# oppo-us-research/PoP-Net

Measured on AMD Instinct MI355X. Metric: depth-frames/sec end-to-end (480x640), higher is better.
Workload: dtype bf16

## Files before the change

popnet_amd/csrc/bb64_kernel.h:

```cpp
#pragma once
#include "conv3_kernel.h"


#define BB_INQ (12 * 32 * 32)
#define BB_IN (4 * BB_INQ)
#define BB_MIDQ (10 * 32 * 32)
#define BB_MID (4 * BB_MIDQ)
#define BB_ASLOT 4096
#define BB_OFF_MID (2 * BB_IN)
#define BB_OFF_A (BB_OFF_MID + BB_MID)
#define BB_NSLOT 6
#define BB_LDS (BB_OFF_A + BB_NSLOT * BB_ASLOT)

typedef __attribute__((ext_vector_type(2))) float f32x2;
typedef __attribute__((ext_vector_type(2))) __bf16 bf16x2;
typedef __attribute__((ext_vector_type(2))) short i16x2;
__device__ __forceinline__ unsigned bb_relu_pk(unsigned w) {
    return __builtin_bit_cast(unsigned, __builtin_elementwise_max(__builtin_bit_cast(i16x2, w), i16x2{0, 0}));
}

template <int HV>
__global__ __launch_bounds__((4 * HV + 4) * 64, 1) void bb64_kernel(const BBProblem P) {
    typedef __bf16 T;
    constexpr int CT = 4 / HV, NCW = 4 * HV, NP = CT / 2, PT1 = 5, PT2 = 4, KK = 9, BQ = 6;
    extern __shared__ __attribute__((aligned(16))) char smem[];
    const int tid = threadIdx.x;
    const int lane = tid & 63;
    const int wave = __builtin_amdgcn_readfirstlane(tid >> 6);
    const int c = lane & 15, q = lane >> 4;
    const int W = P.W, H = P.H;

    volatile int *s_tile = reinterpret_cast<volatile int *>(smem + BB_OFF_MID + 31 * 32);
    const bool dyn = P.tickets != nullptr;
    auto next_tile = [&](int t, int k) -> int { return dyn ? __builtin_amdgcn_readfirstlane(s_tile[(k + 1) & 3]) : t + (int)gridDim.x; };
    auto next_tile_raw = [&](int t, int k) -> int { return dyn ? s_tile[(k + 1) & 3] : t + (int)gridDim.x; };
    auto tile_geom = [&](int t, int &b, int &oy0, int &ox0, int &R, int &Wc) {
        b = t / P.tiles_per_img;
        const int rem = t - b * P.tiles_per_img;
        const int ty = rem / P.tiles_x, tx = rem - ty * P.tiles_x;
        oy0 = ty * 8; ox0 = tx * P.Wt;
        R = min(8, H - oy0); Wc = min(P.Wt, W - ox0);
    };

    if (wave >= NCW) {
        const int lw = wave - NCW;
        const unsigned lane16 = (unsigned)lane * 16u;
        int t = blockIdx.x;
        if (t >= P.ntiles) return;
        if (lw < 2) {
            const char *wsrc = (const char *)P.wpack + lw * 2048;
            auto dma_a = [&](int kstep) {
                pn_glds16_s<0>(wsrc + (size_t)kstep * BB_ASLOT, lane16, (unsigned)(BB_OFF_A + (kstep % BB_NSLOT) * BB_ASLOT) + (unsigned)__builtin_amdgcn_readfirstlane(lw * 2048));
                pn_glds16_s<0>(wsrc + (size_t)kstep * BB_ASLOT + 1024, lane16, (unsigned)(BB_OFF_A + (kstep % BB_NSLOT) * BB_ASLOT + 1024) + (unsigned)__builtin_amdgcn_readfirstlane(lw * 2048));
            };
            dma_a(0); dma_a(1); dma_a(2); dma_a(3);
            asm volatile("s_waitcnt vmcnt(0)\n\ts_barrier" ::: "memory");
            asm volatile("s_barrier" ::: "memory");
            for (int k = 0; t < P.ntiles; ++k) {
                const int tnx = next_tile_raw(t, k);
#pragma clang loop unroll(full)
                for (int p = 0; p < 18; ++p) {
                    dma_a((2 * p + 4) % 36);
                    dma_a((2 * p + 5) % 36);
                    asm volatile("s_waitcnt vmcnt(2)\n\ts_barrier" ::: "memory");
                    if (p == 8) asm volatile("s_barrier" ::: "memory");
                }
                asm volatile("s_barrier" ::: "memory");
                t = __builtin_amdgcn_readfirstlane(tnx);
            }
            asm volatile("s_waitcnt vmcnt(0)" ::: "memory");
            return;
        }
        auto dma_in = [&](int tt, int buf, int n) {
            int b, oy0, ox0, R, Wc;
            tile_geom(tt, b, oy0, ox0, R, Wc);
            const int qu = n / 12, row = n % 12;
            const int px = lane >> 1;
            const int iy = oy0 - 2 + row, ix = ox0 - 2 + px;
            const size_t frame_b = ((size_t)b * H * W * P.in_cs + P.in_coff) * 2;
            const bool inb = px < Wc + 4 && (unsigned)ix < (unsigned)W && (unsigned)iy < (unsigned)H;
            const unsigned off = inb ? (unsigned)((iy * W + ix) * P.in_cs * 2 + qu * 32 + (lane & 1) * 16) : P.in_zero_off - (unsigned)frame_b;
            pn_glds16_s<0>((const char *)P.in + frame_b, off, (unsigned)__builtin_amdgcn_readfirstlane(buf * BB_IN + qu * BB_INQ + row * 1024));
        };
        const int n0 = (lw - 2) * 24;
        const bool ticketer = dyn && lw == 2 && lane == 0;
        int ticket = 0;
        auto claim = [&]() -> int { return 2 * (int)gridDim.x + atomicAdd(P.tickets, 1); };
        if (ticketer) ticket = t + (int)gridDim.x;
#pragma unroll
        for (int j = 0; j < 24; ++j) dma_in(t, 0, n0 + j);
        asm volatile("s_waitcnt vmcnt(0)" ::: "memory");
        if (ticketer) s_tile[1] = ticket;
        asm volatile("s_waitcnt lgkmcnt(0)\n\ts_barrier" ::: "memory");
        asm volatile("s_barrier" ::: "memory");
        int cur = 0;
        for (int k = 0; t < P.ntiles; ++k) {
            const int tnx = next_tile(t, k);
            const int tn = tnx < P.ntiles ? tnx : t;
            int signed_off = -1;
            if (ticketer) {
                if (tnx < P.ntiles) ticket = claim();
                else signed_off = atomicAdd(P.tickets + 1, 1);
            }
#pragma clang loop unroll(full)
            for (int p = 0; p < 18; ++p) {
                if (p < 12) { dma_in(tn, cur ^ 1, n0 + 2 * p); dma_in(tn, cur ^ 1, n0 + 2 * p + 1); }
                asm volatile("s_barrier" ::: "memory");
                if (p == 8) asm volatile("s_barrier" ::: "memory");
            }
            asm volatile("s_waitcnt vmcnt(0)" ::: "memory");
            if (ticketer) {
                s_tile[(k + 2) & 3] = ticket;
                if (signed_off == (int)gridDim.x - 1) {
                    __hip_atomic_store(P.tickets, 0, __ATOMIC_RELAXED, __HIP_MEMORY_SCOPE_AGENT);
                    __hip_atomic_store(P.tickets + 1, 0, __ATOMIC_RELAXED, __HIP_MEMORY_SCOPE_AGENT);
                }
            }
            asm volatile("s_waitcnt lgkmcnt(0)\n\ts_barrier" ::: "memory");
            cur ^= 1;
            t = tnx;
        }
        return;
    }

    int t = blockIdx.x;
    if (t >= P.ntiles) return;
    const float *bias1 = P.bias1, *bias2 = P.bias2;
    const int pw = HV == 2 ? (wave & 3) : wave, hv = HV == 2 ? (wave >> 2) : 0;
    float b1[4 * CT], b2[4 * CT];
#pragma unroll
    for (int i = 0; i < 4 * CT; ++i) { b1[i] = bias1[16 * q + 4 * CT * hv + i]; b2[i] = bias2[16 * q + 4 * CT * hv + i]; }
    const int aaddr = BB_OFF_A + lane * 16 + hv * CT * 1024;
    bf16x8 aq[2][CT], bq[BQ];
    asm volatile("s_barrier" ::: "memory");
#pragma unroll
    for (int ct = 0; ct < CT; ++ct) aq[0][ct] = *reinterpret_cast<const bf16x8 *>(smem + aaddr + ct * 1024);
    asm volatile("s_waitcnt lgkmcnt(0)\n\ts_barrier" ::: "memory");
    int cur = 0;
    for (int it = 0; t < P.ntiles; ++it) {
        const int tnx = next_tile_raw(t, it);
        int b, oy0, ox0, R, Wc;
        tile_geom(t, b, oy0, ox0, R, Wc);
        const int MC = Wc + 2, nmid = (R + 2) * MC, nout = R * Wc;
        const float inv_mc = 1.0f / (float)MC, inv_wc = 1.0f / (float)Wc;
        const int inb = cur * BB_IN;
        int ba1[PT1], ba2[PT2];
#pragma unroll
        for (int pt = 0; pt < PT1; ++pt) {
            const int s0 = (pw * PT1 + pt) * 16 + c, s = s0 < nmid ? s0 : 0;
            const int r = (int)(((float)s + 0.5f) * inv_mc), x = s - r * MC;
            ba1[pt] = inb + (q >> 1) * BB_INQ + (q & 1) * 16 + (r * 32 + x) * 32;
        }
#pragma unroll
        for (int pt = 0; pt < PT2; ++pt) {
            const int s0 = (pw * PT2 + pt) * 16 + c, s = s0 < nout ? s0 : 0;
            const int r = (int)(((float)s + 0.5f) * inv_wc), x = s - r * Wc;
            ba2[pt] = BB_OFF_MID + (q >> 1) * BB_MIDQ + (q & 1) * 16 + (r * 32 + x) * 32;
        }
        f32x4 acc[CT][PT1];
#pragma unroll
        for (int ct = 0; ct < CT; ++ct)
#pragma unroll
            for (int pt = 0; pt < PT1; ++pt) acc[ct][pt] = f32x4{0.f, 0.f, 0.f, 0.f};
#define BB_TAPOFF(tap) ((((tap) / 3) * 32 + ((tap) % 3)) * 32)
#define BB_OFF1(j) ((((j) / PT1) / KK) * 2 * BB_INQ + BB_TAPOFF(((j) / PT1) % KK))
#pragma unroll
        for (int j = 0; j < BQ - 1; ++j) bq[j] = *reinterpret_cast<const bf16x8 *>(smem + ba1[j % PT1] + BB_OFF1(j));
#pragma clang loop unroll(full)
        for (int ph = 0; ph < 18; ++ph) {
            __builtin_amdgcn_sched_barrier(0);
#pragma clang loop unroll(full)
            for (int pt = 0; pt < PT1; ++pt) {
                const int j = ph * PT1 + pt, jr = j + BQ - 1;
                if (pt < CT)
                    aq[(ph + 1) & 1][pt] = *reinterpret_cast<const bf16x8 *>(smem + aaddr + ((ph + 1) % BB_NSLOT) * BB_ASLOT + pt * 1024);
                if (jr < 18 * PT1) bq[jr % BQ] = *reinterpret_cast<const bf16x8 *>(smem + ba1[jr % PT1] + BB_OFF1(jr));
#pragma unroll
                for (int ct = 0; ct < CT; ++ct)
                    acc[ct][pt] = __builtin_amdgcn_mfma_f32_16x16x32_bf16(aq[ph & 1][ct], bq[j % BQ], acc[ct][pt], 0, 0, 0);
                if (pt < CT && jr < 18 * PT1) __builtin_amdgcn_sched_group_barrier(0x100, 2, 0);
                else if (pt < CT || jr < 18 * PT1) __builtin_amdgcn_sched_group_barrier(0x100, 1, 0);
                __builtin_amdgcn_sched_group_barrier(0x008, CT, 0);
            }
            __builtin_amdgcn_sched_barrier(0);
            if (ph & 1) asm volatile("s_barrier" ::: "memory");
        }
#pragma clang loop unroll(full)
        for (int pt = 0; pt < PT1; ++pt) {
            const int s = (pw * PT1 + pt) * 16 + c;
            const int r = (int)(((float)s + 0.5f) * inv_mc), x = s - r * MC;
            const int my = oy0 - 1 + r, mx = ox0 - 1 + x;
            const bool inside = (unsigned)my < (unsigned)H && (unsigned)mx < (unsigned)W;
            const bool border = oy0 == 0 || ox0 == 0 || oy0 + R >= H || ox0 + Wc >= W;
            u32x4 o[NP];
#pragma unroll
            for (int ct = 0; ct < CT; ++ct) {
                f32x2 lo = {acc[ct][pt][0] + b1[4 * ct + 0], acc[ct][pt][1] + b1[4 * ct + 1]};
                f32x2 hi = {acc[ct][pt][2] + b1[4 * ct + 2], acc[ct][pt][3] + b1[4 * ct + 3]};
                o[ct >> 1][2 * (ct & 1)] = bb_relu_pk(__builtin_bit_cast(unsigned, __builtin_convertvector(lo, bf16x2)));
                o[ct >> 1][2 * (ct & 1) + 1] = bb_relu_pk(__builtin_bit_cast(unsigned, __builtin_convertvector(hi, bf16x2)));
            }
            if (border && !inside) {
#pragma unroll
                for (int k = 0; k < NP; ++k) o[k] = u32x4{0u, 0u, 0u, 0u};
            }
            if (s < nmid) {
                u32x4 *dst = reinterpret_cast<u32x4 *>(smem + BB_OFF_MID + q * BB_MIDQ + (r * 32 + x) * 32) + hv * NP;
#pragma unroll
                for (int k = 0; k < NP; ++k) dst[k] = o[k];
            }
        }
        asm volatile("s_waitcnt lgkmcnt(0)\n\ts_barrier" ::: "memory");
#define BB_OFF2(j) ((((j) / PT2) / KK) * 2 * BB_MIDQ + BB_TAPOFF(((j) / PT2) % KK))
#pragma unroll
        for (int ct = 0; ct < CT; ++ct)
#pragma unroll
            for (int pt = 0; pt < PT2; ++pt) acc[ct][pt] = f32x4{0.f, 0.f, 0.f, 0.f};
#pragma unroll
        for (int j = 0; j < BQ - 1; ++j) bq[j] = *reinterpret_cast<const bf16x8 *>(smem + ba2[j % PT2] + BB_OFF2(j));
#pragma clang loop unroll(full)
        for (int p2 = 0; p2 < 18; ++p2) {
            const int ph = 18 + p2;
            __builtin_amdgcn_sched_barrier(0);
#pragma clang loop unroll(full)
            for (int pt = 0; pt < PT2; ++pt) {
                const int j = p2 * PT2 + pt, jr = j + BQ - 1;
                if (pt < CT)
                    aq[(ph + 1) & 1][pt] = *reinterpret_cast<const bf16x8 *>(smem + aaddr + ((ph + 1) % BB_NSLOT) * BB_ASLOT + pt * 1024);
                if (jr < 18 * PT2) bq[jr % BQ] = *reinterpret_cast<const bf16x8 *>(smem + ba2[jr % PT2] + BB_OFF2(jr));
#pragma unroll
                for (int ct = 0; ct < CT; ++ct)
                    acc[ct][pt] = __builtin_amdgcn_mfma_f32_16x16x32_bf16(aq[ph & 1][ct], bq[j % BQ], acc[ct][pt], 0, 0, 0);
                if (pt < CT && jr < 18 * PT2) __builtin_amdgcn_sched_group_barrier(0x100, 2, 0);
                else if (pt < CT || jr < 18 * PT2) __builtin_amdgcn_sched_group_barrier(0x100, 1, 0);
                __builtin_amdgcn_sched_group_barrier(0x008, CT, 0);
            }
            __builtin_amdgcn_sched_barrier(0);
            if (ph & 1) asm volatile("s_barrier" ::: "memory");
        }
        {
            const __amdgpu_buffer_rsrc_t orsrc = __builtin_amdgcn_make_buffer_rsrc(
                (char *)P.out + ((size_t)b * H * W * P.out_cs + P.out_coff) * 2, 0, (int)((size_t)H * W * P.out_cs * 2), 0x00020000);
#pragma clang loop unroll(full)
            for (int pt = 0; pt < PT2; ++pt) {
                const int s = (pw * PT2 + pt) * 16 + c;
                const int r = (int)(((float)s + 0.5f) * inv_wc), x = s - r * Wc;
                const bool valid = s < nout;
                const u32x4 *rp = reinterpret_cast<const u32x4 *>(smem + inb + q * BB_INQ + (((valid ? r : 0) + 2) * 32 + (valid ? x : 0) + 2) * 32);
                u32x4 rr[NP], o[NP];
#pragma unroll
                for (int k = 0; k < NP; ++k) rr[k] = rp[hv * NP + k];
#pragma unroll
                for (int ct = 0; ct < CT; ++ct) {
                    const unsigned ra = rr[ct >> 1][2 * (ct & 1)], rb = rr[ct >> 1][2 * (ct & 1) + 1];
                    f32x2 lo = {acc[ct][pt][0] + b2[4 * ct + 0] + __builtin_bit_cast(float, ra << 16),
                                acc[ct][pt][1] + b2[4 * ct + 1] + __builtin_bit_cast(float, ra & 0xffff0000u)};
                    f32x2 hi = {acc[ct][pt][2] + b2[4 * ct + 2] + __builtin_bit_cast(float, rb << 16),
                                acc[ct][pt][3] + b2[4 * ct + 3] + __builtin_bit_cast(float, rb & 0xffff0000u)};
                    o[ct >> 1][2 * (ct & 1)] = bb_relu_pk(__builtin_bit_cast(unsigned, __builtin_convertvector(lo, bf16x2)));
                    o[ct >> 1][2 * (ct & 1) + 1] = bb_relu_pk(__builtin_bit_cast(unsigned, __builtin_convertvector(hi, bf16x2)));
                }
                const unsigned voff = valid ? (unsigned)(((oy0 + r) * W + ox0 + x) * P.out_cs * 2 + 32 * q) : 0x80000000u;
#pragma unroll
                for (int k = 0; k < NP; ++k) __builtin_amdgcn_raw_buffer_store_b128(o[k], orsrc, voff + 16u * (unsigned)(hv * NP + k), 0, 0);
            }
        }
        asm volatile("s_waitcnt lgkmcnt(0)\n\ts_barrier" ::: "memory");
        cur ^= 1;
        t = __builtin_amdgcn_readfirstlane(tnx);
    }
#undef BB_OFF1
#undef BB_OFF2
#undef BB_TAPOFF
}

static int bb64_launch(pn_ctx *ctx, const BBProblem &P, int num_cus, hipStream_t stream) {
    static PnLdsAttr attr[2];
    const int halves = P.halves == 2 ? 2 : 1;
    if (int rc = pn_lds_attr(ctx, attr[halves - 1], halves == 2 ? reinterpret_cast<const void *>(bb64_kernel<2>) : reinterpret_cast<const void *>(bb64_kernel<1>), BB_LDS)) return rc;
    const int grid = P.ntiles < num_cus ? P.ntiles : num_cus;
    if (halves == 2) hipLaunchKernelGGL(bb64_kernel<2>, dim3(grid), dim3(768), BB_LDS, stream, P);
    else hipLaunchKernelGGL(bb64_kernel<1>, dim3(grid), dim3(512), BB_LDS, stream, P);
    PN_HIP_CHECK(ctx, hipGetLastError());
    return PN_OK;
}
```

Baseline: 69800.

## Overlap conv epilogues with tail MFMAs and rebalance output tiles across waves

For the single-half variant, the last two K-steps of each conv stage are reordered so that each pixel-tile's accumulation finishes early. Its bias/ReLU/store epilogue is then interleaved with the remaining MFMAs through sched_group_barrier fill groups. Output tiles are redistributed so waves split the 4th tile's channels, skipping redundant MFMAs, and biases are staged in LDS instead of held in registers. Address math is simplified with dump pixels and XOR addressing. This adds scheduling complexity and a risk of subtle indexing errors.

```diff
diff --git a/popnet_amd/csrc/bb64_kernel.h b/popnet_amd/csrc/bb64_kernel.h
--- a/popnet_amd/csrc/bb64_kernel.h
+++ b/popnet_amd/csrc/bb64_kernel.h
@@ -11,6 +11,10 @@
 #define BB_OFF_A (BB_OFF_MID + BB_MID)
 #define BB_NSLOT 6
 #define BB_LDS (BB_OFF_A + BB_NSLOT * BB_ASLOT)
+#define BB_BIAS(cv, q) (BB_OFF_MID + (q) * BB_MIDQ + (((cv) + 1) * 32 + 30) * 32)
+
+__host__ __device__ constexpr int bb_item_ks(int n, int PT, bool xch) { return !xch || n < 16 * PT ? n / PT : n - 16 * PT < 4 ? 16 + ((n - 16 * PT) >> 1) : 16 + ((n - 16 * PT) & 1); }
+__host__ __device__ constexpr int bb_item_pt(int n, int PT, bool xch) { return !xch || n < 16 * PT ? n % PT : n - 16 * PT < 4 ? (n - 16 * PT) & 1 : (n - 16 * PT) >> 1; }
 
 typedef __attribute__((ext_vector_type(2))) float f32x2;
 typedef __attribute__((ext_vector_type(2))) __bf16 bf16x2;
@@ -23,6 +27,10 @@
 __global__ __launch_bounds__((4 * HV + 4) * 64, 1) void bb64_kernel(const BBProblem P) {
     typedef __bf16 T;
     constexpr int CT = 4 / HV, NCW = 4 * HV, NP = CT / 2, PT1 = 5, PT2 = 4, KK = 9, BQ = 6;
+    constexpr bool SPLIT = HV == 1;
+    constexpr bool XCH = HV == 1;
+    constexpr int NKO = XCH ? 16 : 18;
+    constexpr int FILL1 = 7, FILL2 = 11;
     extern __shared__ __attribute__((aligned(16))) char smem[];
     const int tid = threadIdx.x;
     const int lane = tid & 63;
@@ -125,16 +133,22 @@
 
     int t = blockIdx.x;
     if (t >= P.ntiles) return;
-    const float *bias1 = P.bias1, *bias2 = P.bias2;
     const int pw = HV == 2 ? (wave & 3) : wave, hv = HV == 2 ? (wave >> 2) : 0;
+    if (wave == 0) {
+        *reinterpret_cast<float *>(smem + BB_BIAS(0, q) + c * 4) = P.bias1[lane];
+        *reinterpret_cast<float *>(smem + BB_BIAS(1, q) + c * 4) = P.bias2[lane];
+    }
+    const int h = SPLIT ? (pw & 1) : 0;
+    auto pct = [&](int i) -> int { return SPLIT ? (i ^ (2 * h)) : hv * CT + i; };
+    auto pc = [&](int k) -> int { return SPLIT ? (k ^ h) : hv * NP + k; };
+    const int biasaddr = BB_BIAS(0, q);
     float b1[4 * CT], b2[4 * CT];
-#pragma unroll
-    for (int i = 0; i < 4 * CT; ++i) { b1[i] = bias1[16 * q + 4 * CT * hv + i]; b2[i] = bias2[16 * q + 4 * CT * hv + i]; }
-    const int aaddr = BB_OFF_A + lane * 16 + hv * CT * 1024;
+    int aaddr0 = BB_OFF_A + lane * 16 + pct(0) * 1024, aaddr1 = aaddr0 ^ 2048;
+    asm volatile("" : "+v"(aaddr0), "+v"(aaddr1));
     bf16x8 aq[2][CT], bq[BQ];
     asm volatile("s_barrier" ::: "memory");
 #pragma unroll
-    for (int ct = 0; ct < CT; ++ct) aq[0][ct] = *reinterpret_cast<const bf16x8 *>(smem + aaddr + ct * 1024);
+    for (int ct = 0; ct < CT; ++ct) aq[0][ct] = *reinterpret_cast<const bf16x8 *>(smem + (ct < 2 ? aaddr0 : aaddr1) + (ct & 1) * 1024);
     asm volatile("s_waitcnt lgkmcnt(0)\n\ts_barrier" ::: "memory");
     int cur = 0;
     for (int it = 0; t < P.ntiles; ++it) {
@@ -144,37 +158,87 @@
         const int MC = Wc + 2, nmid = (R + 2) * MC, nout = R * Wc;
         const float inv_mc = 1.0f / (float)MC, inv_wc = 1.0f / (float)Wc;
         const int inb = cur * BB_IN;
+        auto out_tile = [&](int pt) -> int { return !SPLIT ? pw * PT2 + pt : pt < 3 ? pw * 3 + pt : 12 + (pw >> 1); };
+        int cc = c;
+        asm volatile("" : "+v"(cc));
+        const float fc = (float)cc + 0.5f;
+        const int ba1base = inb + (q >> 1) * BB_INQ + (q & 1) * 16, ba2base = BB_OFF_MID + (q >> 1) * BB_MIDQ + (q & 1) * 16;
+        const int dumppix = (3 * 32 + 30 + (cc & 1)) * 32;
         int ba1[PT1], ba2[PT2];
 #pragma unroll
         for (int pt = 0; pt < PT1; ++pt) {
-            const int s0 = (pw * PT1 + pt) * 16 + c, s = s0 < nmid ? s0 : 0;
-            const int r = (int)(((float)s + 0.5f) * inv_mc), x = s - r * MC;
-            ba1[pt] = inb + (q >> 1) * BB_INQ + (q & 1) * 16 + (r * 32 + x) * 32;
+            const int sb = (pw * PT1 + pt) * 16, s = sb + cc;
+            const int r = (int)((fc + (float)sb) * inv_mc), x = s - r * MC;
+            ba1[pt] = ba1base + (s < nmid ? (r * 32 + x) * 32 : dumppix);
         }
 #pragma unroll
         for (int pt = 0; pt < PT2; ++pt) {
-            const int s0 = (pw * PT2 + pt) * 16 + c, s = s0 < nout ? s0 : 0;
-            const int r = (int)(((float)s + 0.5f) * inv_wc), x = s - r * Wc;
-            ba2[pt] = BB_OFF_MID + (q >> 1) * BB_MIDQ + (q & 1) * 16 + (r * 32 + x) * 32;
+            const int sb = out_tile(pt) * 16, s = sb + cc;
+            const int r = (int)((fc + (float)sb) * inv_wc), x = s - r * Wc;
+            ba2[pt] = ba2base + (s < nout ? (r * 32 + x) * 32 : 0);
         }
         f32x4 acc[CT][PT1];
 #pragma unroll
         for (int ct = 0; ct < CT; ++ct)
 #pragma unroll
             for (int pt = 0; pt < PT1; ++pt) acc[ct][pt] = f32x4{0.f, 0.f, 0.f, 0.f};
+        const bool border = oy0 == 0 || ox0 == 0 || oy0 + R >= H || ox0 + Wc >= W;
+        const int midw = BB_OFF_MID + q * BB_MIDQ + 16 * pc(0);
+        auto epi1 = [&](int pt) {
+            const int pix = ba1[pt] - ba1base, r = pix >> 10, x = (pix >> 5) & 31;
+            const bool inside = (unsigned)(oy0 - 1 + r) < (unsigned)H && (unsigned)(ox0 - 1 + x) < (unsigned)W;
+            const unsigned keep = !border || inside ? 0xffffffffu : 0u;
+            u32x4 o[NP];
+#pragma unroll
+            for (int ct = 0; ct < CT; ++ct) {
+                f32x2 lo = {acc[ct][pt][0] + b1[4 * ct + 0], acc[ct][pt][1] + b1[4 * ct + 1]};
+                f32x2 hi = {acc[ct][pt][2] + b1[4 * ct + 2], acc[ct][pt][3] + b1[4 * ct + 3]};
+                o[ct >> 1][2 * (ct & 1)] = bb_relu_pk(__builtin_bit_cast(unsigned, __builtin_convertvector(lo, bf16x2))) & keep;
+                o[ct >> 1][2 * (ct & 1) + 1] = bb_relu_pk(__builtin_bit_cast(unsigned, __builtin_convertvector(hi, bf16x2))) & keep;
+            }
+            const int dsta = midw + pix;
+            *reinterpret_cast<u32x4 *>(smem + dsta) = o[0];
+            if (NP == 2) *reinterpret_cast<u32x4 *>(smem + (dsta ^ 16)) = o[NP - 1];
+        };
+        const int resw = inb + q * BB_INQ + (2 * 32 + 2) * 32 + 16 * pc(0);
+        __amdgpu_buffer_rsrc_t orsrc;
+        auto epi2 = [&](int pt) {
+            const int nct = SPLIT && pt == 3 ? 2 : CT, np = nct / 2;
+            const int pix = ba2[pt] - ba2base, r = pix >> 10, x = (pix >> 5) & 31;
+            const bool valid = out_tile(pt) * 16 + cc < nout;
+            u32x4 rr[NP], o[NP];
+            rr[0] = *reinterpret_cast<const u32x4 *>(smem + resw + pix);
+            if (np == 2) rr[NP - 1] = *reinterpret_cast<const u32x4 *>(smem + ((resw + pix) ^ 16));
+#pragma unroll
+            for (int ct = 0; ct < nct; ++ct) {
+                const unsigned ra = rr[ct >> 1][2 * (ct & 1)], rb = rr[ct >> 1][2 * (ct & 1) + 1];
+                f32x2 lo = {acc[ct][pt][0] + b2[4 * ct + 0] + __builtin_bit_cast(float, ra << 16),
+                            acc[ct][pt][1] + b2[4 * ct + 1] + __builtin_bit_cast(float, ra & 0xffff0000u)};
+                f32x2 hi = {acc[ct][pt][2] + b2[4 * ct + 2] + __builtin_bit_cast(float, rb << 16),
+                            acc[ct][pt][3] + b2[4 * ct + 3] + __builtin_bit_cast(float, rb & 0xffff0000u)};
+                o[ct >> 1][2 * (ct & 1)] = bb_relu_pk(__builtin_bit_cast(unsigned, __builtin_convertvector(lo, bf16x2)));
+                o[ct >> 1][2 * (ct & 1) + 1] = bb_relu_pk(__builtin_bit_cast(unsigned, __builtin_convertvector(hi, bf16x2)));
+            }
+            unsigned vin = (unsigned)(((oy0 + r) * W + ox0 + x) * P.out_cs * 2 + 32 * q);
+            asm volatile("" : "+v"(vin));
+            const unsigned voff = valid ? vin : 0x80000000u;
+#pragma unroll
+            for (int k = 0; k < np; ++k) __builtin_amdgcn_raw_buffer_store_b128(o[k], orsrc, voff + 16u * (unsigned)pc(k), 0, 0);
+        };
 #define BB_TAPOFF(tap) ((((tap) / 3) * 32 + ((tap) % 3)) * 32)
-#define BB_OFF1(j) ((((j) / PT1) / KK) * 2 * BB_INQ + BB_TAPOFF(((j) / PT1) % KK))
-#pragma unroll
-        for (int j = 0; j < BQ - 1; ++j) bq[j] = *reinterpret_cast<const bf16x8 *>(smem + ba1[j % PT1] + BB_OFF1(j));
-#pragma clang loop unroll(full)
-        for (int ph = 0; ph < 18; ++ph) {
+#define BB_A(k, ct) (*reinterpret_cast<const bf16x8 *>(smem + ((ct) < 2 ? aaddr0 : aaddr1) + ((k) % BB_NSLOT) * BB_ASLOT + ((ct) & 1) * 1024))
+#define BB_KOFF1(ks) (((ks) / KK) * 2 * BB_INQ + BB_TAPOFF((ks) % KK))
+#define BB_B1(n) (*reinterpret_cast<const bf16x8 *>(smem + ba1[bb_item_pt(n, PT1, XCH)] + BB_KOFF1(bb_item_ks(n, PT1, XCH))))
+#pragma unroll
+        for (int j = 0; j < BQ - 1; ++j) bq[j] = BB_B1(j);
+#pragma clang loop unroll(full)
+        for (int ph = 0; ph < NKO; ++ph) {
             __builtin_amdgcn_sched_barrier(0);
 #pragma clang loop unroll(full)
             for (int pt = 0; pt < PT1; ++pt) {
                 const int j = ph * PT1 + pt, jr = j + BQ - 1;
-                if (pt < CT)
-                    aq[(ph + 1) & 1][pt] = *reinterpret_cast<const bf16x8 *>(smem + aaddr + ((ph + 1) % BB_NSLOT) * BB_ASLOT + pt * 1024);
-                if (jr < 18 * PT1) bq[jr % BQ] = *reinterpret_cast<const bf16x8 *>(smem + ba1[jr % PT1] + BB_OFF1(jr));
+                if (pt < CT) aq[(ph + 1) & 1][pt] = BB_A(ph + 1, pt);
+                if (jr < 18 * PT1) bq[jr % BQ] = BB_B1(jr);
 #pragma unroll
                 for (int ct = 0; ct < CT; ++ct)
                     acc[ct][pt] = __builtin_amdgcn_mfma_f32_16x16x32_bf16(aq[ph & 1][ct], bq[j % BQ], acc[ct][pt], 0, 0, 0);
@@ -185,92 +249,115 @@
             __builtin_amdgcn_sched_barrier(0);
             if (ph & 1) asm volatile("s_barrier" ::: "memory");
         }
-#pragma clang loop unroll(full)
-        for (int pt = 0; pt < PT1; ++pt) {
-            const int s = (pw * PT1 + pt) * 16 + c;
-            const int r = (int)(((float)s + 0.5f) * inv_mc), x = s - r * MC;
-            const int my = oy0 - 1 + r, mx = ox0 - 1 + x;
-            const bool inside = (unsigned)my < (unsigned)H && (unsigned)mx < (unsigned)W;
-            const bool border = oy0 == 0 || ox0 == 0 || oy0 + R >= H || ox0 + Wc >= W;
-            u32x4 o[NP];
-#pragma unroll
-            for (int ct = 0; ct < CT; ++ct) {
-                f32x2 lo = {acc[ct][pt][0] + b1[4 * ct + 0], acc[ct][pt][1] + b1[4 * ct + 1]};
-                f32x2 hi = {acc[ct][pt][2] + b1[4 * ct + 2], acc[ct][pt][3] + b1[4 * ct + 3]};
-                o[ct >> 1][2 * (ct & 1)] = bb_relu_pk(__builtin_bit_cast(unsigned, __builtin_convertvector(lo, bf16x2)));
-                o[ct >> 1][2 * (ct & 1) + 1] = bb_relu_pk(__builtin_bit_cast(unsigned, __builtin_convertvector(hi, bf16x2)));
-            }
-            if (border && !inside) {
-#pragma unroll
-                for (int k = 0; k < NP; ++k) o[k] = u32x4{0u, 0u, 0u, 0u};
-            }
-            if (s < nmid) {
-                u32x4 *dst = reinterpret_cast<u32x4 *>(smem + BB_OFF_MID + q * BB_MIDQ + (r * 32 + x) * 32) + hv * NP;
-#pragma unroll
-                for (int k = 0; k < NP; ++k) dst[k] = o[k];
-            }
+#pragma unroll
+        for (int i = 0; i < CT; ++i) *reinterpret_cast<f32x4 *>(b1 + 4 * i) = *reinterpret_cast<const f32x4 *>(smem + biasaddr + 16 * pct(i));
+        if constexpr (XCH) {
+            __builtin_amdgcn_sched_barrier(0);
+#pragma unroll
+            for (int ct = 0; ct < CT; ++ct) aq[1][ct] = BB_A(17, ct);
+#pragma clang loop unroll(full)
+            for (int m = 0; m < 2 * PT1; ++m) {
+                const int n = 16 * PT1 + m, nr = n + BQ - 1, pt = bb_item_pt(n, PT1, true), ks = bb_item_ks(n, PT1, true);
+                if (nr < 18 * PT1) bq[nr % BQ] = BB_B1(nr);
+#pragma unroll
+                for (int ct = 0; ct < CT; ++ct)
+                    acc[ct][pt] = __builtin_amdgcn_mfma_f32_16x16x32_bf16(aq[ks & 1][ct], bq[n % BQ], acc[ct][pt], 0, 0, 0);
+                if (m == 2 * PT1 - 2) {
+#pragma unroll
+                    for (int ct = 0; ct < CT; ++ct) aq[0][ct] = BB_A(18, ct);
+                }
+                if (ks == 17 && pt < PT1 - 1) epi1(pt);
+                if (m == 0) __builtin_amdgcn_sched_group_barrier(0x100, CT + 1, 0);
+                else if (nr < 18 * PT1) __builtin_amdgcn_sched_group_barrier(0x100, 1, 0);
+#pragma unroll
+                for (int ct = 0; ct < CT; ++ct) {
+                    __builtin_amdgcn_sched_group_barrier(0x008, 1, 0);
+                    if (m >= 3) __builtin_amdgcn_sched_group_barrier(0x206, FILL1, 0);
+                }
+                if (m == 2 * PT1 - 2) __builtin_amdgcn_sched_group_barrier(0x100, CT, 0);
+            }
+            __builtin_amdgcn_sched_barrier(0);
+            asm volatile("s_barrier" ::: "memory");
+            epi1(PT1 - 1);
+        } else {
+#pragma clang loop unroll(full)
+            for (int pt = 0; pt < PT1; ++pt) epi1(pt);
         }
         asm volatile("s_waitcnt lgkmcnt(0)\n\ts_barrier" ::: "memory");
-#define BB_OFF2(j) ((((j) / PT2) / KK) * 2 * BB_MIDQ + BB_TAPOFF(((j) / PT2) % KK))
+#define BB_KOFF2(ks) (((ks) / KK) * 2 * BB_MIDQ + BB_TAPOFF((ks) % KK))
+#define BB_B2(n) (*reinterpret_cast<const bf16x8 *>(smem + ba2[bb_item_pt(n, PT2, XCH)] + BB_KOFF2(bb_item_ks(n, PT2, XCH))))
 #pragma unroll
         for (int ct = 0; ct < CT; ++ct)
 #pragma unroll
             for (int pt = 0; pt < PT2; ++pt) acc[ct][pt] = f32x4{0.f, 0.f, 0.f, 0.f};
 #pragma unroll
-        for (int j = 0; j < BQ - 1; ++j) bq[j] = *reinterpret_cast<const bf16x8 *>(smem + ba2[j % PT2] + BB_OFF2(j));
-#pragma clang loop unroll(full)
-        for (int p2 = 0; p2 < 18; ++p2) {
+        for (int j = 0; j < BQ - 1; ++j) bq[j] = BB_B2(j);
+#pragma clang loop unroll(full)
+        for (int p2 = 0; p2 < NKO; ++p2) {
             const int ph = 18 + p2;
             __builtin_amdgcn_sched_barrier(0);
 #pragma clang loop unroll(full)
             for (int pt = 0; pt < PT2; ++pt) {
                 const int j = p2 * PT2 + pt, jr = j + BQ - 1;
-                if (pt < CT)
-                    aq[(ph + 1) & 1][pt] = *reinterpret_cast<const bf16x8 *>(smem + aaddr + ((ph + 1) % BB_NSLOT) * BB_ASLOT + pt * 1024);
-                if (jr < 18 * PT2) bq[jr % BQ] = *reinterpret_cast<const bf16x8 *>(smem + ba2[jr % PT2] + BB_OFF2(jr));
-#pragma unroll
-                for (int ct = 0; ct < CT; ++ct)
+                if (pt < CT) aq[(ph + 1) & 1][pt] = BB_A(ph + 1, pt);
+                if (jr < 18 * PT2) bq[jr % BQ] = BB_B2(jr);
+                const int nct = SPLIT && pt == 3 ? 2 : CT;
+#pragma unroll
+                for (int ct = 0; ct < nct; ++ct)
                     acc[ct][pt] = __builtin_amdgcn_mfma_f32_16x16x32_bf16(aq[ph & 1][ct], bq[j % BQ], acc[ct][pt], 0, 0, 0);
                 if (pt < CT && jr < 18 * PT2) __builtin_amdgcn_sched_group_barrier(0x100, 2, 0);
                 else if (pt < CT || jr < 18 * PT2) __builtin_amdgcn_sched_group_barrier(0x100, 1, 0);
-                __builtin_amdgcn_sched_group_barrier(0x008, CT, 0);
+                if (SPLIT && pt == 3) __builtin_amdgcn_sched_group_barrier(0x008, 2, 0);
+                else __builtin_amdgcn_sched_group_barrier(0x008, CT, 0);
             }
             __builtin_amdgcn_sched_barrier(0);
             if (ph & 1) asm volatile("s_barrier" ::: "memory");
         }
-        {
-            const __amdgpu_buffer_rsrc_t orsrc = __builtin_amdgcn_make_buffer_rsrc(
-                (char *)P.out + ((size_t)b * H * W * P.out_cs + P.out_coff) * 2, 0, (int)((size_t)H * W * P.out_cs * 2), 0x00020000);
-#pragma clang loop unroll(full)
-            for (int pt = 0; pt < PT2; ++pt) {
-                const int s = (pw * PT2 + pt) * 16 + c;
-                const int r = (int)(((float)s + 0.5f) * inv_wc), x = s - r * Wc;
-                const bool valid = s < nout;
-                const u32x4 *rp = reinterpret_cast<const u32x4 *>(smem + inb + q * BB_INQ + (((valid ? r : 0) + 2) * 32 + (valid ? x : 0) + 2) * 32);
-                u32x4 rr[NP], o[NP];
-#pragma unroll
-                for (int k = 0; k < NP; ++k) rr[k] = rp[hv * NP + k];
-#pragma unroll
-                for (int ct = 0; ct < CT; ++ct) {
-                    const unsigned ra = rr[ct >> 1][2 * (ct & 1)], rb = rr[ct >> 1][2 * (ct & 1) + 1];
-                    f32x2 lo = {acc[ct][pt][0] + b2[4 * ct + 0] + __builtin_bit_cast(float, ra << 16),
-                                acc[ct][pt][1] + b2[4 * ct + 1] + __builtin_bit_cast(float, ra & 0xffff0000u)};
-                    f32x2 hi = {acc[ct][pt][2] + b2[4 * ct + 2] + __builtin_bit_cast(float, rb << 16),
-                                acc[ct][pt][3] + b2[4 * ct + 3] + __builtin_bit_cast(float, rb & 0xffff0000u)};
-                    o[ct >> 1][2 * (ct & 1)] = bb_relu_pk(__builtin_bit_cast(unsigned, __builtin_convertvector(lo, bf16x2)));
-                    o[ct >> 1][2 * (ct & 1) + 1] = bb_relu_pk(__builtin_bit_cast(unsigned, __builtin_convertvector(hi, bf16x2)));
-                }
-                const unsigned voff = valid ? (unsigned)(((oy0 + r) * W + ox0 + x) * P.out_cs * 2 + 32 * q) : 0x80000000u;
-#pragma unroll
-                for (int k = 0; k < NP; ++k) __builtin_amdgcn_raw_buffer_store_b128(o[k], orsrc, voff + 16u * (unsigned)(hv * NP + k), 0, 0);
-            }
+#pragma unroll
+        for (int i = 0; i < CT; ++i) *reinterpret_cast<f32x4 *>(b2 + 4 * i) = *reinterpret_cast<const f32x4 *>(smem + biasaddr + 1024 + 16 * pct(i));
+        orsrc = __builtin_amdgcn_make_buffer_rsrc((char *)P.out + ((size_t)b * H * W * P.out_cs + P.out_coff) * 2, 0, (int)((size_t)H * W * P.out_cs * 2), 0x00020000);
+        if constexpr (XCH) {
+            __builtin_amdgcn_sched_barrier(0);
+#pragma unroll
+            for (int ct = 0; ct < CT; ++ct) aq[1][ct] = BB_A(35, ct);
+#pragma clang loop unroll(full)
+            for (int m = 0; m < 2 * PT2; ++m) {
+                const int n = 16 * PT2 + m, nr = n + BQ - 1, pt = bb_item_pt(n, PT2, true), ks = bb_item_ks(n, PT2, true);
+                const int nct = pt == 3 ? 2 : CT;
+                if (nr < 18 * PT2) bq[nr % BQ] = BB_B2(nr);
+#pragma unroll
+                for (int ct = 0; ct < nct; ++ct)
+                    acc[ct][pt] = __builtin_amdgcn_mfma_f32_16x16x32_bf16(aq[ks & 1][ct], bq[n % BQ], acc[ct][pt], 0, 0, 0);
+                if (m == 2 * PT2 - 2) {
+#pragma unroll
+                    for (int ct = 0; ct < CT; ++ct) aq[0][ct] = BB_A(36, ct);
+                }
+                if (ks == 17 && pt < PT2 - 1) epi2(pt);
+                if (m == 0) __builtin_amdgcn_sched_group_barrier(0x100, CT + 1, 0);
+                else if (nr < 18 * PT2) __builtin_amdgcn_sched_group_barrier(0x100, 1, 0);
+#pragma unroll
+                for (int ct = 0; ct < nct; ++ct) {
+                    __builtin_amdgcn_sched_group_barrier(0x008, 1, 0);
+                    if (m >= 3) __builtin_amdgcn_sched_group_barrier(0x146, FILL2, 0);
+                }
+                if (m == 2 * PT2 - 2) __builtin_amdgcn_sched_group_barrier(0x100, CT, 0);
+            }
+            __builtin_amdgcn_sched_barrier(0);
+            asm volatile("s_barrier" ::: "memory");
+            epi2(PT2 - 1);
+        } else {
+#pragma clang loop unroll(full)
+            for (int pt = 0; pt < PT2; ++pt) epi2(pt);
         }
         asm volatile("s_waitcnt lgkmcnt(0)\n\ts_barrier" ::: "memory");
         cur ^= 1;
         t = __builtin_amdgcn_readfirstlane(tnx);
     }
-#undef BB_OFF1
-#undef BB_OFF2
+#undef BB_A
+#undef BB_B1
+#undef BB_B2
+#undef BB_KOFF1
+#undef BB_KOFF2
 #undef BB_TAPOFF
 }
 
```

New measurement: 70740, median of 6. 1.01x the previous value.
